# serycjon/MFT

Hardware: AMD Instinct MI355X
Metric: tracked frames/sec at 512x512, 12 RAFT iters; flow EPE vs reference (higher is better)
Workload: dtype f32 (update-block products as split fp16 x 3 on the fp16 matrix cores, fp32 accumulation; error per product <= ~2^-23, see DESIGN.md section 4 and parity below); 1 GPU; MFT.track on synthetic 512x512 video, deltas [inf,1,2,4,8,16,32], 7/7.00/7 (min/mean/max) flow pairs per timed frame, 12 RAFT iters, seeded synthetic weights (BASELINE.json configs[1]); parallelism=single GPU, frames_resident_in_hbm=True, preroll_frames=32

## Files before the change

include/mftx.h:

```cpp
#ifndef MFTX_H
#define MFTX_H

#include <stddef.h>
#include <stdint.h>

#ifdef __cplusplus
extern "C" {
#endif

#define MFTX_VERSION 400

#define MFTX_E_ARG (-1)
#define MFTX_E_ALIGN (-2)
#define MFTX_E_WORKSPACE (-3)
#define MFTX_E_STATE (-4)

#define MFTX_MAX_CANDIDATES 16

int mftx_version(void);
const char *mftx_last_error_string(void);

#define MFTX_PROFILE_CATEGORIES 14
int mftx_profile_begin(void);
int mftx_profile_end(double *ms, double *work, long long *count, int n);
// ... 31 lines not shown
    float *out; int ldo;
    int P, h, w;
    int N;
    int kh, kw;
    int act;
    float out_scale;
    const float *addend; int ld_addend;
    int stride, hin, win, pad_y, pad_x, residual_mode;
    int arith;
    int a_split, out_split;
} mftx_conv_desc;
#define MFTX_ARITH_F32 0
#define MFTX_ARITH_SPLIT 1
int mftx_conv2d(const mftx_conv_desc *d, void *stream);
int mftx_conv2d_tile(const mftx_conv_desc *d, int tile, void *stream);

int mftx_pack_tile_conv_weights(const float *wpk, int N, int taps, int cin, int cin_pad, void *wtile, void *stream);
int mftx_tile_conv2d(const mftx_conv_desc *d, const void *wtile, void *stream);
#define MFTX_OU_HEADS_WTILE_BYTES 6635520
int mftx_pack_ou_heads_weights(const float *w1pk, int cin_pad, const float *w2pk, void *wtile, void *wproj, void *stream);
int mftx_ou_heads(const float *a_split, int lda, int P, int h, int w, const void *wtile, const float *b1, const void *wproj, const float *b2,
                  float *T, float *out, int ld_out, void *stream);
int mftx_gru_half(const float *h_in, int ld_hin, const float *motion, int ld_mo, const void *wzr, const void *wq, const float *pre_zr,
                  const float *pre_q, float *z, const float *hf_in, float *hf_out, float *h_out, int ld_hout, int P, int h, int w, int pass,
                  void *stream);
int mftx_tile_conv_fills_chip(int P, int h, int w);
#define MFTX_FLOW_HEAD_WEIGHT_BYTES 32768
int mftx_pack_flow_head_weights(const float *w2pk, void *wproj, void *stream);
int mftx_flow_head(const float *hsplit, int ld_h, int P, int h, int w, const void *wtile, const float *b1, const void *wproj,
                   const float *b2, float *T, float *delta, float *coords, void *stream);
// ... 60 lines not shown
                               const float *const *fmap2, const float *const *net, const float *const *inp,
                               const float *const *ctx_parts, const void *const *fmap1_split, const void *fmap2_split,
                               const float *flow_init, int pad_left, int pad_right, int pad_top, int pad_bottom,
                               float *flow, float *occl, float *sigma, float *packed, float *flow_lr_out,
                               void *workspace, size_t workspace_bytes, void *stream);
int mftx_volume_query_split(const float *in, void *out, long long n_floats, void *stream);

typedef struct mftx_encoder mftx_encoder;
int mftx_encoder_create(const float *const *weights, int n_weights, int instance_norm, mftx_encoder **out);
int mftx_encoder_set_split_weights(mftx_encoder *e, const void *const *split, int n);
int mftx_encoder_set_graph(mftx_encoder *e, int on);
void mftx_encoder_destroy(mftx_encoder *e);
size_t mftx_encoder_workspace_bytes(int H0, int W0);
int mftx_encoder_forward(mftx_encoder *e, const uint8_t *img, int H0, int W0, float *out0, float *out1,
                         void *workspace, size_t workspace_bytes, void *stream);
int mftx_encoder_prep(const uint8_t *img, int H0, int W0, float *out, void *stream);
size_t mftx_instance_norm_workspace_bytes(int C);
int mftx_instance_norm(float *x, int rows, int C, const float *res, int mode, int split, void *workspace,
                       size_t workspace_bytes, void *stream);

int mftx_convex_upsample(const float *flow_lr, const float *ou, int ld_ou, const float *mask,
                         int P, int h, int w,
                         int pad_left, int pad_right, int pad_top, int pad_bottom,
                         float *flow, float *occl, float *sigma, float *packed, void *stream);

int mftx_chain(const float *flowL, const float *occlL, const float *sigmaL,
               const float *flowR, const float *occlR, const float *sigmaR,
               int H, int W, float *flowO, float *occlO, float *sigmaO, void *stream);

int mftx_warp_backward(const float *flow, const float *img, int C, int H, int W, float *out, void *stream);
// ... 98 lines not shown
```

mft_amd/_lib.py:

```python
from __future__ import annotations

import ctypes as C
import os
from pathlib import Path

_HERE = Path(__file__).resolve().parent
LIB_PATH = _HERE / "libmftx.so"

MAX_CANDIDATES = 16
NUM_RAFT_WEIGHTS = 34
LOOKUP_CONVC1_WEIGHT_BYTES = 393216
FLOW_BRANCH_WEIGHT_BYTES = 352256
FLOW_HEAD_WEIGHT_BYTES = 32768
OU_HEADS_WTILE_BYTES = 6635520
SPLIT_LIMIT = 65504.0


class ConvDesc(C.Structure):
    _fields_ = [("a0", C.c_void_p), ("lda0", C.c_int), ("c0", C.c_int),
                ("a1", C.c_void_p), ("lda1", C.c_int), ("c1", C.c_int),
                ("wpk", C.c_void_p), ("bias", C.c_void_p),
                ("out", C.c_void_p), ("ldo", C.c_int),
                ("P", C.c_int), ("h", C.c_int), ("w", C.c_int),
                ("N", C.c_int), ("kh", C.c_int), ("kw", C.c_int),
# ... 10 lines not shown
    "mftx_last_error_string": (C.c_char_p, []),
    "mftx_profile_begin": (C.c_int, []),
    "mftx_profile_end": (C.c_int, [C.POINTER(C.c_double), C.POINTER(C.c_double), C.POINTER(C.c_longlong), C.c_int]),
    "mftx_corr_pyramid": (C.c_int, [C.c_void_p, C.c_void_p, C.c_int, C.c_int, C.c_int, C.c_int,
                                    C.c_void_p, C.c_void_p, C.c_void_p, C.c_void_p, C.c_void_p]),
    "mftx_corr_pyramid_split": (C.c_int, [C.c_void_p, C.c_void_p, C.c_int, C.c_int, C.c_int, C.c_int,
                                          C.c_void_p, C.c_void_p, C.c_void_p, C.c_void_p, C.c_void_p, C.c_void_p]),
    "mftx_corr_pyramid_layout": (C.c_int, [C.c_int, C.c_int, C.POINTER(C.c_longlong), C.POINTER(C.c_int)]),
    "mftx_corr_lookup": (C.c_int, [C.c_void_p] * 5 + [C.c_int] * 4 + [C.c_void_p, C.c_int, C.c_void_p]),
    "mftx_fmap_pyramid": (C.c_int, [C.c_void_p] + [C.c_int] * 4 + [C.c_void_p] * 4),
    "mftx_corr_lookup_ondemand": (C.c_int, [C.c_void_p] * 6 + [C.c_int] * 5 + [C.c_void_p, C.c_int, C.c_void_p]),
    "mftx_raft_set_ondemand": (C.c_int, [C.c_void_p, C.c_int]),
    "mftx_raft_workspace_bytes_for": (C.c_size_t, [C.c_void_p, C.c_int, C.c_int, C.c_int]),
    "mftx_conv2d": (C.c_int, [C.POINTER(ConvDesc), C.c_void_p]),
    "mftx_conv2d_tile": (C.c_int, [C.POINTER(ConvDesc), C.c_int, C.c_void_p]),
    "mftx_encoder_set_split_weights": (C.c_int, [C.c_void_p, _PP, C.c_int]),
    "mftx_raft_set_split_weights": (C.c_int, [C.c_void_p, _PP, C.c_int]),
    "mftx_raft_arith": (C.c_int, [C.c_void_p]),
    "mftx_raft_set_lookup_fused": (C.c_int, [C.c_void_p, C.c_void_p]),
    "mftx_raft_set_flow_fused": (C.c_int, [C.c_void_p, C.c_void_p]),
    "mftx_raft_set_tile_weights": (C.c_int, [C.c_void_p, _PP, C.c_int]),
    "mftx_raft_set_flow_head": (C.c_int, [C.c_void_p, C.c_void_p]),
    "mftx_raft_set_ou_heads": (C.c_int, [C.c_void_p, C.c_void_p, C.c_void_p]),
    "mftx_pack_ou_heads_weights": (C.c_int, [C.c_void_p, C.c_int, C.c_void_p, C.c_void_p, C.c_void_p, C.c_void_p]),
    "mftx_ou_heads": (C.c_int, [C.c_void_p, C.c_int, C.c_int, C.c_int, C.c_int, C.c_void_p, C.c_void_p, C.c_void_p, C.c_void_p, C.c_void_p,
                                C.c_void_p, C.c_int, C.c_void_p]),
    "mftx_pack_flow_head_weights": (C.c_int, [C.c_void_p, C.c_void_p, C.c_void_p]),
    "mftx_flow_head": (C.c_int, [C.c_void_p, C.c_int, C.c_int, C.c_int, C.c_int] + [C.c_void_p] * 8),
    "mftx_pack_tile_conv_weights": (C.c_int, [C.c_void_p, C.c_int, C.c_int, C.c_int, C.c_int, C.c_void_p, C.c_void_p]),
    "mftx_tile_conv2d": (C.c_int, [C.POINTER(ConvDesc), C.c_void_p, C.c_void_p]),
# ... 31 lines not shown
                                          C.c_void_p, C.c_size_t, C.c_void_p]),
    "mftx_raft_refine_gather_ex": (C.c_int, [C.c_void_p, C.c_int, C.c_int, C.c_int, C.c_int,
                                             _PP, _PP, _PP, _PP, _PP, _PP, C.c_void_p, C.c_void_p,
                                             C.c_int, C.c_int, C.c_int, C.c_int,
                                             C.c_void_p, C.c_void_p, C.c_void_p, C.c_void_p, C.c_void_p,
                                             C.c_void_p, C.c_size_t, C.c_void_p]),
    "mftx_raft_frame_prepare_bytes": (C.c_size_t, [C.c_int, C.c_int]),
    "mftx_raft_frame_prepare": (C.c_int, [C.c_void_p, C.c_int, C.c_int] + [C.c_void_p] * 8 + [C.c_size_t, C.c_void_p]),
    "mftx_volume_query_split": (C.c_int, [C.c_void_p, C.c_void_p, C.c_longlong, C.c_void_p]),
    "mftx_encoder_create": (C.c_int, [_PP, C.c_int, C.c_int, C.POINTER(C.c_void_p)]),
    "mftx_encoder_destroy": (None, [C.c_void_p]),
    "mftx_encoder_set_graph": (C.c_int, [C.c_void_p, C.c_int]),
    "mftx_encoder_workspace_bytes": (C.c_size_t, [C.c_int, C.c_int]),
    "mftx_encoder_forward": (C.c_int, [C.c_void_p, C.c_void_p, C.c_int, C.c_int, C.c_void_p, C.c_void_p,
                                       C.c_void_p, C.c_size_t, C.c_void_p]),
    "mftx_encoder_prep": (C.c_int, [C.c_void_p, C.c_int, C.c_int, C.c_void_p, C.c_void_p]),
    "mftx_instance_norm_workspace_bytes": (C.c_size_t, [C.c_int]),
    "mftx_instance_norm": (C.c_int, [C.c_void_p, C.c_int, C.c_int, C.c_void_p, C.c_int, C.c_int, C.c_void_p, C.c_size_t, C.c_void_p]),
    "mftx_convex_upsample": (C.c_int, [C.c_void_p, C.c_void_p, C.c_int, C.c_void_p] + [C.c_int] * 7
                             + [C.c_void_p] * 5),
    "mftx_chain": (C.c_int, [C.c_void_p] * 6 + [C.c_int, C.c_int] + [C.c_void_p] * 4),
    "mftx_warp_backward": (C.c_int, [C.c_void_p, C.c_void_p, C.c_int, C.c_int, C.c_int, C.c_void_p, C.c_void_p]),
    "mftx_select": (C.c_int, [C.c_int, _PP, _PP, _PP, C.c_float, C.c_int, C.c_int] + [C.c_void_p] * 5),
    "mftx_chain_select": (C.c_int, [C.c_int] + [_PP] * 6 + [C.c_float, C.c_int, C.c_int] + [C.c_void_p] * 5),
    "mftx_chain_select_packed": (C.c_int, [C.c_int] + [_PP] * 4 + [C.c_float, C.c_int, C.c_int] + [C.c_void_p] * 5),
    "mftx_chain_select_multi": (C.c_int, [C.c_int, C.POINTER(C.c_int)] + [_PP] * 4 + [C.c_float, C.c_int, C.c_int] + [_PP] * 4
                                + [C.c_void_p]),
    "mftx_sample_points": (C.c_int, [C.c_int, _PP, _PP, _PP, C.c_int, C.c_int, C.c_int, C.c_void_p, C.c_void_p,
                                     C.c_void_p, C.c_longlong, C.c_int, C.c_void_p]),
    "mftx_splat_forward": (C.c_int, [C.c_void_p, C.c_void_p, C.c_int, C.c_void_p, C.c_int, C.c_int, C.c_int, C.c_int, C.c_int,
# ... 67 lines not shown
```

mft_amd/csrc/common.h:

```cpp
#pragma once
#include <hip/hip_runtime.h>
#include <cstdarg>
#include <cstdio>
#include <cstdint>
#include <cstdlib>
#include "../../include/mftx.h"

namespace mftx {

void set_error(const char *fmt, ...);

inline int fail(int code, const char *fmt, ...) {
    char buf[512];
    va_list ap;
    va_start(ap, fmt);
    vsnprintf(buf, sizeof buf, fmt, ap);
    va_end(ap);
    set_error("%s", buf);
    return code;
}

inline int check_launch(const char *what) {
    hipError_t e = hipGetLastError();
    if (e != hipSuccess) {
// ... 58 lines not shown
        const _Float16 b = __builtin_bit_cast(_Float16, (unsigned short)(hi ? ll >> 16 : ll));
        return (float)a + (float)b * (1.f / 2048.f);
    };
    return make_float4(dec(h.x, l.x, 0), dec(h.x, l.x, 1), dec(h.y, l.y, 0), dec(h.y, l.y, 1));
}
__device__ __forceinline__ void store_split4v(float *row, int c, float4 v) {
    const unsigned a = split_halves(v.x), b = split_halves(v.y), cc = split_halves(v.z), d = split_halves(v.w);
    char *dst = reinterpret_cast<char *>(row) + split_row_offset(c);
    *reinterpret_cast<uint2 *>(dst) = make_uint2((a & 0xffffu) | (b << 16), (cc & 0xffffu) | (d << 16));
    *reinterpret_cast<uint2 *>(dst + 16) = make_uint2((a >> 16) | (b & 0xffff0000u), (cc >> 16) | (d & 0xffff0000u));
}
#endif
__host__ __device__ inline float relu_keep_nan(float v) { return v < 0.f ? 0.f : v; }
int launch_conv(const mftx_conv_desc &d, hipStream_t s, int tile = -1);
int launch_conv_pair(const mftx_conv_desc &a, const mftx_conv_desc &b, hipStream_t s);
struct GruEpilogue {
    int mode;
    float *hx;
    int ld_hx;
    float *z;
    float *rh;
    float *hf = nullptr;
    int ld_hf = 0;
};
int launch_conv_gru(const mftx_conv_desc &d, const GruEpilogue &g, hipStream_t s);
int launch_split_weights(const float *wpk, void *out, long long n_floats, hipStream_t s);
bool conv_small_applicable(const mftx_conv_desc &d);
int launch_conv_small(const mftx_conv_desc &d, hipStream_t s, float *accum = nullptr, int ld_accum = 0);
int launch_corr_pyramid(const float *f1, const float *f2, int P, int C, int h, int w, float *const lvl[4], hipStream_t s,
                        float *f2_split = nullptr, int tile_resident = 1);
// ... 64 lines not shown
```

mft_amd/csrc/conv_gemm.hip:

```cpp
#include "common.h"
#include "profile.h"
#include "device_prims.h"
#include <cstdlib>
#include <type_traits>

namespace mftx {

enum Arith { AR_F32 = 0, AR_SPLIT = 1, AR_PRESPLIT = 2 };

#ifdef MFTX_TIMING
__device__ unsigned long long mftx_dbg[16];
#endif
#if defined(MFTX_TIMING) && MFTX_TIMING == 1
#define STAMP(i) asm volatile("s_memtime %0" : "=s"(ts[i]))
#define MFTX_TIMING_LOOP 1
#else
#define STAMP(i)
#endif

constexpr int BK = 32;
constexpr int LDK = BK;
constexpr unsigned OOB = 0x80000000u;

enum Epi { EPI_GENERIC = 0, EPI_RELU = 1, EPI_GRU_ZR = 2, EPI_GRU_Q = 3,
// ... 1291 lines not shown
        hipError_t e = hipFuncSetAttribute(reinterpret_cast<const void *>(kern),
                                           hipFuncAttributeMaxDynamicSharedMemorySize, (int)lds);
        if (e != hipSuccess) return fail((int)e, "hipFuncSetAttribute: %s", hipGetErrorString(e));
        attr_set = true;
    }
    const long long n_virtual = 8ll * cdiv(cdiv(a.M, BM), 8) * cdiv(a.N, BN) + 8ll * cdiv(cdiv(b.M, BM), 8) * cdiv(b.N, BN);
    static const bool one_tile_per_wg = tune_env("MFTX_CONV_NONPERSISTENT", 0) != 0;
    const long long slots = one_tile_per_wg ? n_virtual : (long long)num_cus() * 4;
    dim3 grid((unsigned)(n_virtual < slots ? n_virtual : slots));
    ProfScope prof(PC_CONV_GEMM, s, 2.0 * a.M * a.N * (double)(a.kh * a.kw) * (a.c0 + a.c1) +
                                        2.0 * b.M * b.N * (double)(b.kh * b.kw) * (b.c0 + b.c1));
    hipLaunchKernelGGL(kern, grid, dim3(256), lds, s, a, b);
    return check_launch("conv_gemm pair");
}

int launch_conv_gru(const mftx_conv_desc &d, const GruEpilogue &g, hipStream_t s) {
    if (int e = validate(d)) return e;
    ConvArgs a = to_args(d);
    a.hx = g.hx; a.ld_hx = g.ld_hx; a.z = g.z; a.rh = g.rh;
    a.hf = g.hf ? g.hf : g.hx; a.ld_hf = g.hf ? g.ld_hf : g.ld_hx;
    if ((g.mode == 1 && d.N != 256) || (g.mode == 2 && d.N != 128)) return fail(MFTX_E_ARG, "gru epilogue: bad N");
    return dispatch(a, g.mode == 1 ? EPI_GRU_ZR : EPI_GRU_Q, 1, s, PC_CONV_GEMM);
}

__global__ void split_weights_kernel(const float *__restrict__ in, uint4 *__restrict__ out, long long n8) {
    const long long i = (long long)blockIdx.x * blockDim.x + threadIdx.x;
    if (i >= n8) return;
    _Float16 hi[8], lo[8];
#pragma unroll
    for (int e = 0; e < 8; ++e) {
// ... 58 lines not shown
```

mft_amd/csrc/encoder.hip:

```cpp
#include "common.h"
#include "profile.h"
#include "graph_cache.h"
#include <new>

namespace mftx {


__global__ void enc_prep_kernel(const uint8_t *__restrict__ img, int H0, int W0, int pl, int pt, int Hp, int Wp,
                                float *__restrict__ out) {
    const int xo = blockIdx.x * blockDim.x + threadIdx.x;
    const int y = blockIdx.y;
    if (xo >= Wp + 6) return;
    float4 v = make_float4(0.f, 0.f, 0.f, 0.f);
    const int x = xo - 3;
    if (x >= 0 && x < Wp) {
        const int sy = min(max(y - pt, 0), H0 - 1), sx = min(max(x - pl, 0), W0 - 1);
        const uint8_t *p = img + ((long long)sy * W0 + sx) * 3;
        v.x = 2.f * ((float)p[2] / 255.0f) - 1.0f;
        v.y = 2.f * ((float)p[1] / 255.0f) - 1.0f;
        v.z = 2.f * ((float)p[0] / 255.0f) - 1.0f;
    }
    reinterpret_cast<float4 *>(out)[(long long)y * (Wp + 6) + xo] = v;
}

// ... 174 lines not shown
    return ws;
}

}

using namespace mftx;

struct mftx_encoder {
    uint32_t magic;
    int instance_norm;
    const float *w[EC_COUNT], *b[EC_COUNT];
    const float *wg[EC_COUNT];
    int arith;
    int use_graph;
    GraphCache *graphs;
};
static constexpr uint32_t ENC_MAGIC = 0x454e4358;

extern "C" int mftx_encoder_create(const float *const *weights, int n_weights, int instance_norm, mftx_encoder **out) {
    if (!weights || !out) return fail(MFTX_E_ARG, "encoder_create: null pointer");
    const int n_conv = instance_norm ? EC_COUNT - 1 : EC_COUNT;
    if (n_weights != 2 * n_conv) return fail(MFTX_E_ARG, "encoder_create: expected %d tensors, got %d", 2 * n_conv, n_weights);
    for (int i = 0; i < n_weights; ++i)
        if (!weights[i] || !aligned16(weights[i])) return fail(MFTX_E_ALIGN, "encoder_create: tensor %d null or unaligned", i);
    mftx_encoder *e = new (std::nothrow) mftx_encoder;
    if (!e) return fail(MFTX_E_ARG, "encoder_create: out of host memory");
    e->magic = ENC_MAGIC;
    e->instance_norm = instance_norm ? 1 : 0;
    for (int i = 0; i < EC_COUNT; ++i) { e->w[i] = e->wg[i] = nullptr; e->b[i] = nullptr; }
    for (int i = 0; i < n_conv; ++i) { e->w[i] = e->wg[i] = weights[2 * i]; e->b[i] = weights[2 * i + 1]; }
    e->arith = MFTX_ARITH_F32;
    e->use_graph = 1;
    e->graphs = new (std::nothrow) GraphCache;
    *out = e;
    return 0;
}

extern "C" int mftx_encoder_set_split_weights(mftx_encoder *e, const void *const *split, int n) {
    if (e && e->magic == ENC_MAGIC && e->graphs) e->graphs->clear();
    if (!e || e->magic != ENC_MAGIC) return fail(MFTX_E_STATE, "encoder_set_split_weights: bad handle");
    const int n_conv = e->instance_norm ? EC_COUNT - 1 : EC_COUNT;
    if (!split) {
        for (int i = 0; i < n_conv; ++i) e->wg[i] = e->w[i];
        e->arith = MFTX_ARITH_F32;
        return 0;
    }
    if (n != n_conv) return fail(MFTX_E_ARG, "encoder_set_split_weights: expected %d weights, got %d", n_conv, n);
    for (int i = 0; i < n_conv; ++i)
        if (!split[i] || !aligned16(split[i])) return fail(MFTX_E_ALIGN, "encoder_set_split_weights: weight %d null or unaligned", i);
    for (int i = 0; i < n_conv; ++i) e->wg[i] = static_cast<const float *>(split[i]);
    e->arith = MFTX_ARITH_SPLIT;
    return 0;
}

extern "C" void mftx_encoder_destroy(mftx_encoder *e) {
// ... 6 lines not shown
    return 0;
}

extern "C" size_t mftx_encoder_workspace_bytes(int H0, int W0) {
    if (H0 <= 0 || W0 <= 0) return 0;
    const int Hp = (H0 + 7) / 8 * 8, Wp = (W0 + 7) / 8 * 8;
    return enc_carve(nullptr, Hp, Wp).bytes;
}

namespace {
struct Enc {
    const mftx_encoder *e;
    EncWs ws;
    hipStream_t s;

    int conv(int slot, const float *in, int cin, int lda, int hin, int win, float *out, int cout, int ldo, int h,
             int w, int k, int stride, int act, const float *residual = nullptr, bool a_split = false, bool out_split = false) {
        mftx_conv_desc d{};
        d.a0 = in; d.lda0 = lda; d.c0 = cin;
        d.wpk = e->wg[slot]; d.bias = e->b[slot]; d.arith = e->arith;
        d.a_split = SP() && a_split; d.out_split = SP() && out_split;
        d.out = out; d.ldo = ldo; d.P = 1; d.h = h; d.w = w; d.N = cout; d.kh = k; d.kw = k;
        d.act = act; d.out_scale = 1.f;
        d.stride = stride; d.hin = hin; d.win = win;
        if (residual) { d.addend = residual; d.ld_addend = cout; d.residual_mode = 1; }
        ProfConvCat cat(PC_ENC_GEMM);
        return launch_conv(d, s);
    }
    bool SP() const { return e->arith == MFTX_ARITH_SPLIT; }
    int norm(float *x, int rows, int C, int mode, const float *res = nullptr) {
        return launch_instance_norm(x, rows, C, res, mode, SP() ? 1 : 0, ws.part, ws.stat, s);
    }
    int block(int c1, int c2, int ds, const float *x, int cin, int hin, int win, float *tmp, float *sc, float *out,
              int planes, int h, int w, int stride) {
        const int rows = h * w;
        if (e->instance_norm) {
            TRY(conv(c1, x, cin, cin, hin, win, tmp, planes, planes, h, w, 3, stride, 0, nullptr, true));
            TRY(norm(tmp, rows, planes, 0));
            TRY(conv(c2, tmp, planes, planes, h, w, out, planes, planes, h, w, 3, 1, 0, nullptr, true));
            const float *shortcut = x;
            if (stride != 1) {
                TRY(conv(ds, x, cin, cin, hin, win, sc, planes, planes, h, w, 1, stride, 0, nullptr, true));
// ... 23 lines not shown
    Enc E{e, enc_carve(workspace, Hp, Wp), (hipStream_t)stream};
    if (E.ws.bytes > workspace_bytes) return fail(MFTX_E_WORKSPACE, "encoder_forward: workspace %zu < %zu", workspace_bytes, E.ws.bytes);
    const bool graphs_on = e->graphs && e->use_graph && !prof_enabled();
    bool proxied = false;
    if (graphs_on && E.s == nullptr) {
        hipStream_t own = e->graphs->proxy.enter(nullptr);
        if (own) { E.s = own; proxied = true; }
    }
    struct Leave { GraphCache *g; bool on; ~Leave() { if (on) g->proxy.leave(nullptr); } } leave{e->graphs, proxied};
    hipStream_t s = E.s;
    TRY(launch_enc_prep(img, H0, W0, E.ws.img, s));
    const int h3 = Hp / 8, w3 = Wp / 8;
    auto body = [&]() -> int {
    const int h1 = Hp / 2, w1 = Wp / 2;
    {
        mftx_conv_desc d{};
        d.a0 = E.ws.img; d.lda0 = 4; d.c0 = 28;
        d.wpk = e->wg[EC_STEM]; d.bias = e->b[EC_STEM]; d.arith = e->arith;
        d.out = E.ws.a; d.ldo = 64; d.P = 1; d.h = h1; d.w = w1; d.N = 64; d.kh = 7; d.kw = 1;
        d.act = e->instance_norm ? 0 : 1; d.out_scale = 1.f;
        d.stride = 2; d.hin = Hp; d.win = Wp + 6; d.pad_y = 3; d.pad_x = -1;
        ProfConvCat cat(PC_ENC_GEMM);
        TRY(launch_conv(d, s));
    }
    if (e->instance_norm) TRY(E.norm(E.ws.a, h1 * w1, 64, 0));
    TRY(E.block(EC_L1B0C1, EC_L1B0C2, -1, E.ws.a, 64, h1, w1, E.ws.b, nullptr, E.ws.c, 64, h1, w1, 1));
    TRY(E.block(EC_L1B1C1, EC_L1B1C2, -1, E.ws.c, 64, h1, w1, E.ws.b, nullptr, E.ws.a, 64, h1, w1, 1));
    const int h2 = h1 / 2, w2 = w1 / 2;
    float *sc2 = E.ws.b + (size_t)h2 * w2 * 96;
    TRY(E.block(EC_L2B0C1, EC_L2B0C2, EC_L2B0DS, E.ws.a, 64, h1, w1, E.ws.b, sc2, E.ws.c, 96, h2, w2, 2));
    TRY(E.block(EC_L2B1C1, EC_L2B1C2, -1, E.ws.c, 96, h2, w2, E.ws.b, nullptr, E.ws.a, 96, h2, w2, 1));
    float *sc3 = E.ws.b + (size_t)h3 * w3 * 128;
    TRY(E.block(EC_L3B0C1, EC_L3B0C2, EC_L3B0DS, E.ws.a, 96, h2, w2, E.ws.b, sc3, E.ws.c, 128, h3, w3, 2));
    return E.block(EC_L3B1C1, EC_L3B1C2, -1, E.ws.c, 128, h3, w3, E.ws.b, nullptr, E.ws.a, 128, h3, w3, 1);
    };
    if (graphs_on) {
        GraphKey key{};
        key.v[0] = (uintptr_t)H0; key.v[1] = (uintptr_t)W0; key.v[2] = reinterpret_cast<uintptr_t>(workspace);
        key.v[3] = reinterpret_cast<uintptr_t>(s); key.v[4] = (uintptr_t)e->arith;
        TRY(e->graphs->run(key, s, body));
    } else {
        TRY(body());
    }
    if (e->instance_norm) return E.conv(EC_HEAD, E.ws.a, 128, 128, h3, w3, out0, 256, 256, h3, w3, 1, 1, 0, nullptr, true);
    TRY(E.conv(EC_HEAD, E.ws.a, 128, 128, h3, w3, out0, 128, 128, h3, w3, 1, 1, 3));
    return E.conv(EC_HEAD2, E.ws.a, 128, 128, h3, w3, out1, 128, 128, h3, w3, 1, 1, 1);
}

extern "C" int mftx_encoder_prep(const uint8_t *img, int H0, int W0, float *out, void *stream) {
    if (!img || !out) return fail(MFTX_E_ARG, "encoder_prep: null pointer");
    if (H0 < 1 || W0 < 1) return fail(MFTX_E_ARG, "encoder_prep: empty image");
    if (!aligned16(out)) return fail(MFTX_E_ALIGN, "encoder_prep: out must be 16-byte aligned");
    return launch_enc_prep(img, H0, W0, out, (hipStream_t)stream);
}

extern "C" size_t mftx_instance_norm_workspace_bytes(int C) {
    if (C < 8 || C > 256 || C % 8) return 0;
    return instnorm_ws_bytes(C);
}

extern "C" int mftx_instance_norm(float *x, int rows, int C, const float *res, int mode, int split, void *workspace,
                                  size_t workspace_bytes, void *stream) {
    if (!x || !workspace) return fail(MFTX_E_ARG, "instance_norm: null pointer");
// ... 15 lines not shown
```

mft_amd/csrc/raft_engine.hip:

```cpp
#include "common.h"
#include "profile.h"
#include "motion_front.h"
#include "graph_cache.h"
#include <cstdlib>
#include <new>

namespace mftx {


struct InitGather { int on; PairPtrs netp, inpp; };
struct CtxTable { const float **table; const float *own[4]; int supplied; PairPtrs parts[4]; };
__global__ void init_state_kernel(const float *__restrict__ net, const float *__restrict__ inp,
                                  const float *__restrict__ flow_init, float *hx, float *hf, float *coords1, int M, int h,
                                  int w, InitGather ga, CtxTable ct) {
    const long long i = (long long)blockIdx.x * blockDim.x + threadIdx.x;
    if (i >= (long long)M * 64) return;
    if (ct.table != nullptr && i < (long long)(M / (h * w)) * 4) {
        const int b = (int)(i >> 2), k = (int)(i & 3);
        ct.table[i] = ct.supplied ? ct.parts[k].p[b] : ct.own[k] + (long long)b * h * w * ((k & 1) ? 128 : 256);
    }
    const int m = (int)(i >> 6), q = (int)(i & 63);
    if (ga.on) {
        const int b = m / (h * w);
        net = ga.netp.p[b] - (long long)b * h * w * 128;
// ... 924 lines not shown
    if (!wpk || !out) return fail(MFTX_E_ARG, "split_weights: null pointer");
    return launch_split_weights(wpk, out, n_floats, (hipStream_t)stream);
}

extern "C" int mftx_conv2d(const mftx_conv_desc *d, void *stream) {
    if (!d) return fail(MFTX_E_ARG, "conv2d: null descriptor");
    return launch_conv(*d, (hipStream_t)stream);
}

extern "C" int mftx_conv2d_tile(const mftx_conv_desc *d, int tile, void *stream) {
    if (!d) return fail(MFTX_E_ARG, "conv2d_tile: null descriptor");
    if (tile < -1 || tile > 15) return fail(MFTX_E_ARG, "conv2d_tile: tile must be -1 (the library's choice) or 0..15");
    return launch_conv(*d, (hipStream_t)stream, tile);
}

extern "C" int mftx_convex_upsample(const float *flow_lr, const float *ou, int ld_ou, const float *mask, int P,
                                    int h, int w, int pad_left, int pad_right, int pad_top, int pad_bottom,
                                    float *flow, float *occl, float *sigma, float *packed, void *stream) {
    const bool planar = flow && occl && sigma;
    if (!flow_lr || !ou || !mask || (!planar && (flow || occl || sigma || !packed)))
        return fail(MFTX_E_ARG, "convex_upsample: null pointer (outputs: flow + occl + sigma, or packed, or both)");
    if (P <= 0 || h <= 0 || w <= 0 || ld_ou < 3) return fail(MFTX_E_ARG, "convex_upsample: bad sizes");
    return launch_convex_upsample(flow_lr, ou, ld_ou, mask, P, h, w, pad_left, pad_right, pad_top, pad_bottom, flow,
                                  occl, sigma, packed, (hipStream_t)stream);
}
```

mft_amd/ops.py:

```python
from __future__ import annotations

import ctypes as C
import math
from typing import NamedTuple

import numpy as np
import torch

from . import _lib
from ._lib import ConvDesc, MftxError, check

ACT = {None: 0, "none": 0, "relu": 1, "sigmoid": 2, "tanh": 3}


def _stream():
    return C.c_void_p(torch.cuda.current_stream().cuda_stream)


def _device_visible(t):
    return isinstance(t, torch.Tensor) and (t.is_cuda or t.is_pinned())


def copy_bytes(src: torch.Tensor, dst: torch.Tensor):
    if not (_device_visible(src) and _device_visible(dst)):
# ... 190 lines not shown
            outs = out
            want = ((h * w, 256), None) if self.instance_norm else ((h * w, 128), (h * w, 128))
            for t, shp in zip(outs, want):
                if shp is not None and (t is None or tuple(t.shape) != shp):
                    raise MftxError(f"encoder output must be {shp}")
        elif self.instance_norm:
            outs = (torch.empty(h * w, 256, dtype=torch.float32, device=self.device), None)
        else:
            outs = (torch.empty(h * w, 128, dtype=torch.float32, device=self.device),
                    torch.empty(h * w, 128, dtype=torch.float32, device=self.device))
        check(lib.mftx_encoder_forward(self._h, _chk(img_u8, "img", torch.uint8), H0, W0, _chk(outs[0], "out0"),
                                       _chk(outs[1], "out1") if outs[1] is not None else None,
                                       self._ws.data_ptr(), self._ws.numel(), _stream()), "mftx_encoder_forward")
        return outs


def encoder_prep(img_u8: torch.Tensor) -> torch.Tensor:
    lib = _lib.load()
    if img_u8.dim() != 3 or img_u8.shape[2] != 3:
        raise MftxError("encoder_prep: img must be [H0, W0, 3]")
    H0, W0 = int(img_u8.shape[0]), int(img_u8.shape[1])
    Hp, Wp = -(-H0 // 8) * 8, -(-W0 // 8) * 8
    out = torch.empty(Hp, Wp + 6, 4, dtype=torch.float32, device=img_u8.device)
    check(lib.mftx_encoder_prep(_chk(img_u8, "img", torch.uint8), H0, W0, out.data_ptr(), _stream()), "mftx_encoder_prep")
    return out


def instance_norm(x: torch.Tensor, mode: int, res: torch.Tensor = None, split: bool = False) -> torch.Tensor:
    lib = _lib.load()
    if x.dim() != 2:
# ... 230 lines not shown


def corr_lookup_ondemand(f1: torch.Tensor, f2_levels, coords: torch.Tensor, h: int, w: int, r: int = 4):
    lib = _lib.load()
    P, N, Cc = f1.shape
    out = torch.empty(P, N, 324, dtype=torch.float32, device=f1.device)
    check(lib.mftx_corr_lookup_ondemand(_chk(f1, "f1"), *[_chk(t, "f2 level") for t in f2_levels], _chk(coords, "coords"),
                                        P, Cc, h, w, r, out.data_ptr(), 324, _stream()), "mftx_corr_lookup_ondemand")
    return out


def conv2d(x: torch.Tensor, wpk: torch.Tensor, bias, P, h, w, N, kh, kw, act=None, out_scale=1.0, x2=None,
           addend=None, stride=0, hin=0, win=0, pad_y=0, pad_x=0, residual_mode=0, arith=ARITH_F32, a_split=False,
           out_split=False, out=None, tile=None, lda0=None, c0=None):
    lib = _lib.load()
    if out is None:
        out = torch.empty(P * h * w, N, dtype=torch.float32, device=x.device)
    d = ConvDesc()
    d.a0, d.lda0, d.c0 = _chk(x, "x"), x.shape[1] if lda0 is None else int(lda0), x.shape[1] if c0 is None else int(c0)
    if x2 is not None:
        d.a1, d.lda1, d.c1 = _chk(x2, "x2"), x2.shape[1], x2.shape[1]
    else:
        d.a1, d.lda1, d.c1 = None, 0, 0
    d.wpk = _chk(wpk, "wpk")
    d.bias = _chk(bias, "bias") if bias is not None else None
    d.out, d.ldo = _chk(out, "out"), out.shape[1]
    d.P, d.h, d.w, d.N, d.kh, d.kw = P, h, w, N, kh, kw
    d.act, d.out_scale = ACT[act], out_scale
    d.addend, d.ld_addend = (_chk(addend, "addend"), addend.shape[1]) if addend is not None else (None, 0)
    d.stride, d.hin, d.win, d.pad_y, d.pad_x, d.residual_mode = stride, hin, win, pad_y, pad_x, residual_mode
    d.arith = arith
    d.a_split, d.out_split = int(bool(a_split)), int(bool(out_split))
    if tile is None:
        check(lib.mftx_conv2d(C.byref(d), _stream()), "mftx_conv2d")
    else:
        check(lib.mftx_conv2d_tile(C.byref(d), int(tile), _stream()), "mftx_conv2d_tile")
    return out


def convex_upsample(flow_lr, ou, mask, P, h, w, pads=(0, 0, 0, 0), want_packed=False):
    lib = _lib.load()
    pl, pr, pt, pb = pads
    H0, W0 = 8 * h - pt - pb, 8 * w - pl - pr
    dev = flow_lr.device
    flow = torch.empty(P, 2, H0, W0, dtype=torch.float32, device=dev)
    occl = torch.empty(P, 1, H0, W0, dtype=torch.float32, device=dev)
    sigma = torch.empty(P, 1, H0, W0, dtype=torch.float32, device=dev)
    packed = torch.empty(P, H0, W0, 4, dtype=torch.float32, device=dev) if want_packed else None
    check(lib.mftx_convex_upsample(_chk(flow_lr, "flow_lr"), _chk(ou, "ou"), ou.shape[1], _chk(mask, "mask"),
                                   P, h, w, pl, pr, pt, pb, flow.data_ptr(), occl.data_ptr(), sigma.data_ptr(),
                                   packed.data_ptr() if want_packed else None, _stream()), "mftx_convex_upsample")
    return (flow, occl, sigma, packed) if want_packed else (flow, occl, sigma)
# ... 755 lines not shown
```

mft_amd/raft.py:

```python
from __future__ import annotations

import logging
import os
from pathlib import Path

import numpy as np
import torch
import torch.nn.functional as F

from . import ops
from .weights import make_weights, strip_module_prefix

logger = logging.getLogger(__name__)


def pad_amounts(H0, W0):
    ph = (((H0 // 8) + 1) * 8 - H0) % 8
    pw = (((W0 // 8) + 1) * 8 - W0) % 8
    return pw // 2, pw - pw // 2, ph // 2, ph - ph // 2


_STREAMS = {}


def _shared_stream(device, kind, index=0):
# ... 47 lines not shown
            self._build_engines()
        self._check_finite = bool(getattr(getattr(config, "raft_params", None), "check_finite", False))
        self._split_streams = int(os.environ.get("MFTX_SPLIT_STREAMS", "") or getattr(config, "split_streams", 0) or
                                  (1 if self._arith == ops.ARITH_SPLIT else 2))
        self._engines, self._side = [], []
        self._fif = self._frames_in_flight_setting(config)
        self._lanes, self._lane_next = [], 0
        self._lanes_stale = False
        self._ahead_max = max(2, int(getattr(config, "max_batches_ahead", 0) or 16))
        self._ahead = []
        self.nominal_pairs = int(getattr(config, "nominal_pairs", 0) or 7)
        self._tile_choice = {}
        fp = os.environ.get("MFTX_FRAME_PREPARE", "")
        self._frame_prepare = bool(int(fp)) if fp else bool(getattr(config, "__dict__", {}).get("frame_prepare", True))
        self._prepare_ok = {}
        self._frames = {}
        self._staging = {}
        ae = getattr(config, "__dict__", {}).get("async_encode", None)
        self._enc_waits_for_device_frames = ae is None
        if ae is None:
            ae = self._frames_in_flight_setting(config) > 1
        self._enc_stream = _shared_stream(self.device, "enc") if ae else None

    def _frames_in_flight_setting(self, config):
        return max(1, int(os.environ.get("MFTX_FRAMES_IN_FLIGHT", "") or getattr(config, "frames_in_flight", 0) or
                          (2 if self._arith == ops.ARITH_SPLIT else 1)))

    def _build_engines(self):
        graph = bool(self._engine_options.get("graph", 1))
        self.fnet_engine = ops.EncoderEngine(self.sd, "fnet", True, self.device, arith=self._arith, graph=graph)
# ... 157 lines not shown
            ring["slots"].append(slot)
        else:
            slot = ring["slots"][ring["n"] % self.STAGING_SLOTS]
        ring["n"] += 1
        if slot[1] is not None:
            slot[1].synchronize()
            slot[1] = None
        np.copyto(slot[0].numpy(), img.numpy() if img.is_contiguous() else np.ascontiguousarray(img.numpy()))
        return slot[0]

    @torch.no_grad()
    def encode(self, img_bgr, want_context=True) -> FrameFeatures:
        H0, W0 = img_bgr.shape[:2]
        img = self._device_image(img_bgr)
        h, w, pads = self._geometry(H0, W0)
        fmap, _ = self.fnet_engine.forward(img)
        net = inp = None
        if want_context:
            net, inp = self.cnet_engine.forward(img)
        return FrameFeatures(fmap, net, inp, h, w, pads, (H0, W0))

    def ensure_encode_stream(self):
        if self._enc_stream is None:
            self._enc_stream = _shared_stream(self.device, "enc")
            self._enc_stream.wait_stream(torch.cuda.current_stream(self.device))
        return self._enc_stream

    @torch.no_grad()
    def encode_packed(self, img_bgr, wait=True):
        H0, W0 = img_bgr.shape[:2]
        h, w, _ = self._geometry(H0, W0)
        N = h * w

        def run():
            img = self._device_image(img_bgr)
            buf = torch.empty(N * 512, dtype=torch.float32, device=self.device)
            self.fnet_engine.forward(img, out=(buf[: N * 256].view(N, 256), None))
            self.cnet_engine.forward(img, out=(buf[N * 256: N * 384].view(N, 128), buf[N * 384:].view(N, 128)))
            return buf

        if self._enc_stream is None or torch.cuda.current_stream(self.device) == self._enc_stream:
            cur = torch.cuda.current_stream(self.device)
            self._encode_begin(cur)
            buf = run()
            self._encode_end(cur.record_event(), cur)
            return buf, (h, w)
        main = torch.cuda.current_stream(self.device)
        self._encode_begin(self._enc_stream)
        with torch.cuda.stream(self._enc_stream):
            buf = run()
            self._encode_end(self._enc_stream.record_event(), self._enc_stream)
        if wait:
            main.wait_stream(self._enc_stream)
# ... 282 lines not shown
```

Measured before the change: 191.6 frames/s.

## Run fnet and cnet encoders together via grouped conv launches

Adds a grouped conv GEMM kernel that runs up to four independent split-arithmetic convolutions in one launch, each member taking its own virtual-tile range. A new paired encoder path interleaves the fnet and cnet layers so matching convolutions of both encoders share a launch, and the pair is captured as one graph. The aim is fewer launches and better CU fill for the small per-frame encoder convs. Members that do not fit the 64x64 tile fall back to separate launches, and the two graph caches now key on a per-encoder generation counter.

Measured after the change: 191.9 frames/s (median of 6 runs). Within noise of the previous version (+0.2%).

```diff
diff --git a/include/mftx.h b/include/mftx.h
--- a/include/mftx.h
+++ b/include/mftx.h
@@ -69,6 +69,7 @@
 #define MFTX_ARITH_SPLIT 1
 int mftx_conv2d(const mftx_conv_desc *d, void *stream);
 int mftx_conv2d_tile(const mftx_conv_desc *d, int tile, void *stream);
+int mftx_conv2d_group(const mftx_conv_desc *d, int n, void *stream);
 
 int mftx_pack_tile_conv_weights(const float *wpk, int N, int taps, int cin, int cin_pad, void *wtile, void *stream);
 int mftx_tile_conv2d(const mftx_conv_desc *d, const void *wtile, void *stream);
@@ -159,6 +160,9 @@
 size_t mftx_encoder_workspace_bytes(int H0, int W0);
 int mftx_encoder_forward(mftx_encoder *e, const uint8_t *img, int H0, int W0, float *out0, float *out1,
                          void *workspace, size_t workspace_bytes, void *stream);
+int mftx_encoder_forward_pair(mftx_encoder *fnet, mftx_encoder *cnet, const uint8_t *img, int H0, int W0, float *fmap,
+                              float *net, float *inp, void *ws_f, size_t ws_f_bytes, void *ws_c, size_t ws_c_bytes,
+                              void *stream);
 int mftx_encoder_prep(const uint8_t *img, int H0, int W0, float *out, void *stream);
 size_t mftx_instance_norm_workspace_bytes(int C);
 int mftx_instance_norm(float *x, int rows, int C, const float *res, int mode, int split, void *workspace,
diff --git a/mft_amd/_lib.py b/mft_amd/_lib.py
--- a/mft_amd/_lib.py
+++ b/mft_amd/_lib.py
@@ -48,6 +48,7 @@
     "mftx_raft_workspace_bytes_for": (C.c_size_t, [C.c_void_p, C.c_int, C.c_int, C.c_int]),
     "mftx_conv2d": (C.c_int, [C.POINTER(ConvDesc), C.c_void_p]),
     "mftx_conv2d_tile": (C.c_int, [C.POINTER(ConvDesc), C.c_int, C.c_void_p]),
+    "mftx_conv2d_group": (C.c_int, [C.POINTER(ConvDesc), C.c_int, C.c_void_p]),
     "mftx_encoder_set_split_weights": (C.c_int, [C.c_void_p, _PP, C.c_int]),
     "mftx_raft_set_split_weights": (C.c_int, [C.c_void_p, _PP, C.c_int]),
     "mftx_raft_arith": (C.c_int, [C.c_void_p]),
@@ -109,6 +110,8 @@
     "mftx_encoder_workspace_bytes": (C.c_size_t, [C.c_int, C.c_int]),
     "mftx_encoder_forward": (C.c_int, [C.c_void_p, C.c_void_p, C.c_int, C.c_int, C.c_void_p, C.c_void_p,
                                        C.c_void_p, C.c_size_t, C.c_void_p]),
+    "mftx_encoder_forward_pair": (C.c_int, [C.c_void_p, C.c_void_p, C.c_void_p, C.c_int, C.c_int, C.c_void_p, C.c_void_p,
+                                            C.c_void_p, C.c_void_p, C.c_size_t, C.c_void_p, C.c_size_t, C.c_void_p]),
     "mftx_encoder_prep": (C.c_int, [C.c_void_p, C.c_int, C.c_int, C.c_void_p, C.c_void_p]),
     "mftx_instance_norm_workspace_bytes": (C.c_size_t, [C.c_int]),
     "mftx_instance_norm": (C.c_int, [C.c_void_p, C.c_int, C.c_int, C.c_void_p, C.c_int, C.c_int, C.c_void_p, C.c_size_t, C.c_void_p]),
diff --git a/mft_amd/csrc/common.h b/mft_amd/csrc/common.h
--- a/mft_amd/csrc/common.h
+++ b/mft_amd/csrc/common.h
@@ -96,6 +96,9 @@
 __host__ __device__ inline float relu_keep_nan(float v) { return v < 0.f ? 0.f : v; }
 int launch_conv(const mftx_conv_desc &d, hipStream_t s, int tile = -1);
 int launch_conv_pair(const mftx_conv_desc &a, const mftx_conv_desc &b, hipStream_t s);
+constexpr int CONV_GROUP_MAX = 4;
+bool conv_group_member_ok(const mftx_conv_desc &d);
+int launch_conv_group(const mftx_conv_desc *d, int n, hipStream_t s);
 struct GruEpilogue {
     int mode;
     float *hx;
diff --git a/mft_amd/csrc/conv_gemm.hip b/mft_amd/csrc/conv_gemm.hip
--- a/mft_amd/csrc/conv_gemm.hip
+++ b/mft_amd/csrc/conv_gemm.hip
@@ -1329,6 +1329,60 @@
     return check_launch("conv_gemm pair");
 }
 
+struct ConvGroupArgs { ConvArgs m[CONV_GROUP_MAX]; int n; };
+
+__global__ __launch_bounds__(256, min_waves_split(1, 4))
+void conv_gemm_group_kernel(ConvGroupArgs g) {
+    int before = 0;
+#pragma unroll 1
+    for (int i = 0; i < g.n; ++i) {
+        const ConvArgs &p = g.m[i];
+        int vt = (int)blockIdx.x - before % (int)gridDim.x;
+        if (vt < 0) vt += gridDim.x;
+        if (p.a_pre) conv_gemm_body<64, 64, 2, 2, EPI_GENERIC, 32, AR_PRESPLIT, 3>(p, vt);
+        else conv_gemm_body<64, 64, 2, 2, EPI_GENERIC, 32, AR_SPLIT, 3>(p, vt);
+        before += n_virtual_tiles(p, 64, 64);
+    }
+}
+
+bool conv_group_member_ok(const mftx_conv_desc &d) {
+    if (d.arith != AR_SPLIT || d.P <= 0 || d.h <= 0 || d.w <= 0 || d.N <= 0) return false;
+    if (d.addend == nullptr && d.stride <= 1 && d.hin == 0 && conv_small_applicable(d)) return false;
+    return pick_tile(to_args(d), 1, -1) == 9;
+}
+
+int launch_conv_group(const mftx_conv_desc *d, int n, hipStream_t s) {
+    if (!d || n < 2 || n > CONV_GROUP_MAX) return fail(MFTX_E_ARG, "conv group: 2..%d members", CONV_GROUP_MAX);
+    ConvGroupArgs g{};
+    g.n = n;
+    long long n_virtual = 0;
+    double work = 0.0;
+    for (int i = 0; i < n; ++i) {
+        if (int e = validate(d[i])) return e;
+        if (!conv_group_member_ok(d[i]))
+            return fail(MFTX_E_ARG, "conv group: member %d does not run on the split arithmetic's 64 x 64 tile", i);
+        ConvArgs &a = g.m[i];
+        a = to_args(d[i]);
+        a.batch = 1;
+        n_virtual += 8ll * cdiv(cdiv(a.M, 64), 8) * cdiv(a.N, 64);
+        work += 2.0 * a.M * a.N * (double)(a.kh * a.kw) * (a.c0 + a.c1);
+    }
+    if (n_virtual > 0x7fffffffLL) return fail(MFTX_E_ARG, "conv group: too many tiles");
+    constexpr size_t lds = (size_t)3 * (64 + 64) * LDK * sizeof(float);
+    static bool attr_set = false;
+    if (!attr_set) {
+        hipError_t e = hipFuncSetAttribute(reinterpret_cast<const void *>(conv_gemm_group_kernel),
+                                           hipFuncAttributeMaxDynamicSharedMemorySize, (int)lds);
+        if (e != hipSuccess) return fail((int)e, "hipFuncSetAttribute: %s", hipGetErrorString(e));
+        attr_set = true;
+    }
+    const long long slots = (long long)num_cus() * 3;
+    dim3 grid((unsigned)(n_virtual < slots ? n_virtual : slots));
+    ProfScope prof(PC_CONV_GEMM, s, work);
+    hipLaunchKernelGGL(conv_gemm_group_kernel, grid, dim3(256), lds, s, g);
+    return check_launch("conv_gemm group");
+}
+
 int launch_conv_gru(const mftx_conv_desc &d, const GruEpilogue &g, hipStream_t s) {
     if (int e = validate(d)) return e;
     ConvArgs a = to_args(d);
diff --git a/mft_amd/csrc/encoder.hip b/mft_amd/csrc/encoder.hip
--- a/mft_amd/csrc/encoder.hip
+++ b/mft_amd/csrc/encoder.hip
@@ -1,6 +1,7 @@
 #include "common.h"
 #include "profile.h"
 #include "graph_cache.h"
+#include <atomic>
 #include <new>
 
 namespace mftx {
@@ -212,8 +213,10 @@
     int arith;
     int use_graph;
     GraphCache *graphs;
+    unsigned long long gen;
 };
 static constexpr uint32_t ENC_MAGIC = 0x454e4358;
+static unsigned long long enc_next_gen() { static std::atomic<unsigned long long> g{0}; return ++g; }
 
 extern "C" int mftx_encoder_create(const float *const *weights, int n_weights, int instance_norm, mftx_encoder **out) {
     if (!weights || !out) return fail(MFTX_E_ARG, "encoder_create: null pointer");
@@ -230,6 +233,7 @@
     e->arith = MFTX_ARITH_F32;
     e->use_graph = 1;
     e->graphs = new (std::nothrow) GraphCache;
+    e->gen = enc_next_gen();
     *out = e;
     return 0;
 }
@@ -237,6 +241,7 @@
 extern "C" int mftx_encoder_set_split_weights(mftx_encoder *e, const void *const *split, int n) {
     if (e && e->magic == ENC_MAGIC && e->graphs) e->graphs->clear();
     if (!e || e->magic != ENC_MAGIC) return fail(MFTX_E_STATE, "encoder_set_split_weights: bad handle");
+    e->gen = enc_next_gen();
     const int n_conv = e->instance_norm ? EC_COUNT - 1 : EC_COUNT;
     if (!split) {
         for (int i = 0; i < n_conv; ++i) e->wg[i] = e->w[i];
@@ -273,8 +278,9 @@
     EncWs ws;
     hipStream_t s;
 
-    int conv(int slot, const float *in, int cin, int lda, int hin, int win, float *out, int cout, int ldo, int h,
-             int w, int k, int stride, int act, const float *residual = nullptr, bool a_split = false, bool out_split = false) {
+    mftx_conv_desc desc(int slot, const float *in, int cin, int lda, int hin, int win, float *out, int cout, int ldo, int h,
+                        int w, int k, int stride, int act, const float *residual = nullptr, bool a_split = false,
+                        bool out_split = false) const {
         mftx_conv_desc d{};
         d.a0 = in; d.lda0 = lda; d.c0 = cin;
         d.wpk = e->wg[slot]; d.bias = e->b[slot]; d.arith = e->arith;
@@ -283,8 +289,22 @@
         d.act = act; d.out_scale = 1.f;
         d.stride = stride; d.hin = hin; d.win = win;
         if (residual) { d.addend = residual; d.ld_addend = cout; d.residual_mode = 1; }
+        return d;
+    }
+    int conv(int slot, const float *in, int cin, int lda, int hin, int win, float *out, int cout, int ldo, int h,
+             int w, int k, int stride, int act, const float *residual = nullptr, bool a_split = false, bool out_split = false) {
+        const mftx_conv_desc d = desc(slot, in, cin, lda, hin, win, out, cout, ldo, h, w, k, stride, act, residual, a_split, out_split);
         ProfConvCat cat(PC_ENC_GEMM);
         return launch_conv(d, s);
+    }
+    mftx_conv_desc stem_desc(const float *img, int Hp, int Wp) const {
+        mftx_conv_desc d{};
+        d.a0 = img; d.lda0 = 4; d.c0 = 28;
+        d.wpk = e->wg[EC_STEM]; d.bias = e->b[EC_STEM]; d.arith = e->arith;
+        d.out = ws.a; d.ldo = 64; d.P = 1; d.h = Hp / 2; d.w = Wp / 2; d.N = 64; d.kh = 7; d.kw = 1;
+        d.act = e->instance_norm ? 0 : 1; d.out_scale = 1.f;
+        d.stride = 2; d.hin = Hp; d.win = Wp + 6; d.pad_y = 3; d.pad_x = -1;
+        return d;
     }
     bool SP() const { return e->arith == MFTX_ARITH_SPLIT; }
     int norm(float *x, int rows, int C, int mode, const float *res = nullptr) {
@@ -338,12 +358,7 @@
     auto body = [&]() -> int {
     const int h1 = Hp / 2, w1 = Wp / 2;
     {
-        mftx_conv_desc d{};
-        d.a0 = E.ws.img; d.lda0 = 4; d.c0 = 28;
-        d.wpk = e->wg[EC_STEM]; d.bias = e->b[EC_STEM]; d.arith = e->arith;
-        d.out = E.ws.a; d.ldo = 64; d.P = 1; d.h = h1; d.w = w1; d.N = 64; d.kh = 7; d.kw = 1;
-        d.act = e->instance_norm ? 0 : 1; d.out_scale = 1.f;
-        d.stride = 2; d.hin = Hp; d.win = Wp + 6; d.pad_y = 3; d.pad_x = -1;
+        const mftx_conv_desc d = E.stem_desc(E.ws.img, Hp, Wp);
         ProfConvCat cat(PC_ENC_GEMM);
         TRY(launch_conv(d, s));
     }
@@ -371,6 +386,100 @@
     return E.conv(EC_HEAD2, E.ws.a, 128, 128, h3, w3, out1, 128, 128, h3, w3, 1, 1, 1);
 }
 
+namespace {
+struct EncPair {
+    Enc F, C;
+    hipStream_t s;
+
+    int group(const mftx_conv_desc *d, int n) {
+        ProfConvCat cat(PC_ENC_GEMM);
+        bool ok = n >= 2;
+        for (int i = 0; i < n; ++i) ok = ok && conv_group_member_ok(d[i]);
+        if (ok) return launch_conv_group(d, n, s);
+        for (int i = 0; i < n; ++i) TRY(launch_conv(d[i], s));
+        return 0;
+    }
+    int block(int c1, int c2, int ds, float *EncWs::*x, int cin, int hin, int win, size_t sc_off, float *EncWs::*out, int planes,
+              int h, int w, int stride) {
+        const int rows = h * w;
+        const float *xf = F.ws.*x, *xc = C.ws.*x;
+        float *tf = F.ws.b, *tc = C.ws.b, *sf = F.ws.b + sc_off, *sc = C.ws.b + sc_off, *of = F.ws.*out, *oc = C.ws.*out;
+        mftx_conv_desc d[4];
+        int n = 0;
+        d[n++] = F.desc(c1, xf, cin, cin, hin, win, tf, planes, planes, h, w, 3, stride, 0, nullptr, true);
+        d[n++] = C.desc(c1, xc, cin, cin, hin, win, tc, planes, planes, h, w, 3, stride, 1, nullptr, false, true);
+        if (stride != 1) {
+            d[n++] = F.desc(ds, xf, cin, cin, hin, win, sf, planes, planes, h, w, 1, stride, 0, nullptr, true);
+            d[n++] = C.desc(ds, xc, cin, cin, hin, win, sc, planes, planes, h, w, 1, stride, 0);
+        }
+        TRY(group(d, n));
+        TRY(F.norm(tf, rows, planes, 0));
+        d[0] = F.desc(c2, tf, planes, planes, h, w, of, planes, planes, h, w, 3, 1, 0, nullptr, true);
+        d[1] = C.desc(c2, tc, planes, planes, h, w, oc, planes, planes, h, w, 3, 1, 1, stride != 1 ? sc : xc, true);
+        TRY(group(d, 2));
+        if (stride != 1) TRY(F.norm(sf, rows, planes, 2));
+        return F.norm(of, rows, planes, 1, stride != 1 ? sf : xf);
+    }
+};
+}
+
+extern "C" int mftx_encoder_forward_pair(mftx_encoder *f, mftx_encoder *c, const uint8_t *img, int H0, int W0, float *fmap,
+                                         float *net, float *inp, void *ws_f, size_t ws_f_bytes, void *ws_c, size_t ws_c_bytes,
+                                         void *stream) {
+    if (!f || f->magic != ENC_MAGIC || !c || c->magic != ENC_MAGIC) return fail(MFTX_E_STATE, "encoder_forward_pair: bad handle");
+    if (!f->instance_norm || c->instance_norm) return fail(MFTX_E_ARG, "encoder_forward_pair: fnet (instance norm) first, then cnet");
+    if (f->arith != MFTX_ARITH_SPLIT || c->arith != MFTX_ARITH_SPLIT)
+        return fail(MFTX_E_ARG, "encoder_forward_pair: both encoders must run the split arithmetic");
+    if (!img || !fmap || !net || !inp || !ws_f || !ws_c) return fail(MFTX_E_ARG, "encoder_forward_pair: null pointer");
+    if (ws_f == ws_c) return fail(MFTX_E_ARG, "encoder_forward_pair: the two workspaces must differ");
+    if (H0 < 16 || W0 < 16) return fail(MFTX_E_ARG, "encoder_forward_pair: image too small");
+    if ((reinterpret_cast<uintptr_t>(ws_f) | reinterpret_cast<uintptr_t>(ws_c)) & 255)
+        return fail(MFTX_E_ALIGN, "encoder_forward_pair: workspaces must be 256-byte aligned");
+    if (prof_enabled()) {
+        TRY(mftx_encoder_forward(f, img, H0, W0, fmap, nullptr, ws_f, ws_f_bytes, stream));
+        return mftx_encoder_forward(c, img, H0, W0, net, inp, ws_c, ws_c_bytes, stream);
+    }
+    const int Hp = enc_pad(H0, W0).Hp, Wp = enc_pad(H0, W0).Wp;
+    EncPair P{Enc{f, enc_carve(ws_f, Hp, Wp), (hipStream_t)stream}, Enc{c, enc_carve(ws_c, Hp, Wp), (hipStream_t)stream}, (hipStream_t)stream};
+    if (P.F.ws.bytes > ws_f_bytes || P.C.ws.bytes > ws_c_bytes)
+        return fail(MFTX_E_WORKSPACE, "encoder_forward_pair: workspace %zu / %zu < %zu", ws_f_bytes, ws_c_bytes, P.F.ws.bytes);
+    const bool graphs_on = f->graphs && f->use_graph && c->use_graph;
+    bool proxied = false;
+    if (graphs_on && P.s == nullptr) {
+        hipStream_t own = f->graphs->proxy.enter(nullptr);
+        if (own) { P.s = P.F.s = P.C.s = own; proxied = true; }
+    }
+    struct Leave { GraphCache *g; bool on; ~Leave() { if (on) g->proxy.leave(nullptr); } } leave{f->graphs, proxied};
+    hipStream_t s = P.s;
+    TRY(launch_enc_prep(img, H0, W0, P.F.ws.img, s));
+    const int h1 = Hp / 2, w1 = Wp / 2, h2 = h1 / 2, w2 = w1 / 2, h3 = Hp / 8, w3 = Wp / 8;
+    auto body = [&]() -> int {
+        mftx_conv_desc d[2] = {P.F.stem_desc(P.F.ws.img, Hp, Wp), P.C.stem_desc(P.F.ws.img, Hp, Wp)};
+        TRY(P.group(d, 2));
+        TRY(P.F.norm(P.F.ws.a, h1 * w1, 64, 0));
+        TRY(P.block(EC_L1B0C1, EC_L1B0C2, -1, &EncWs::a, 64, h1, w1, 0, &EncWs::c, 64, h1, w1, 1));
+        TRY(P.block(EC_L1B1C1, EC_L1B1C2, -1, &EncWs::c, 64, h1, w1, 0, &EncWs::a, 64, h1, w1, 1));
+        TRY(P.block(EC_L2B0C1, EC_L2B0C2, EC_L2B0DS, &EncWs::a, 64, h1, w1, (size_t)h2 * w2 * 96, &EncWs::c, 96, h2, w2, 2));
+        TRY(P.block(EC_L2B1C1, EC_L2B1C2, -1, &EncWs::c, 96, h2, w2, 0, &EncWs::a, 96, h2, w2, 1));
+        TRY(P.block(EC_L3B0C1, EC_L3B0C2, EC_L3B0DS, &EncWs::a, 96, h2, w2, (size_t)h3 * w3 * 128, &EncWs::c, 128, h3, w3, 2));
+        return P.block(EC_L3B1C1, EC_L3B1C2, -1, &EncWs::c, 128, h3, w3, 0, &EncWs::a, 128, h3, w3, 1);
+    };
+    if (graphs_on) {
+        GraphKey key{};
+        key.v[0] = (uintptr_t)H0; key.v[1] = (uintptr_t)W0; key.v[2] = reinterpret_cast<uintptr_t>(ws_f);
+        key.v[3] = reinterpret_cast<uintptr_t>(s); key.v[4] = (uintptr_t)f->arith;
+        key.v[5] = reinterpret_cast<uintptr_t>(c); key.v[6] = (uintptr_t)c->gen; key.v[7] = reinterpret_cast<uintptr_t>(ws_c);
+        key.v[8] = 1;
+        TRY(f->graphs->run(key, s, body));
+    } else {
+        TRY(body());
+    }
+    mftx_conv_desc d[3] = {P.F.desc(EC_HEAD, P.F.ws.a, 128, 128, h3, w3, fmap, 256, 256, h3, w3, 1, 1, 0, nullptr, true),
+                           P.C.desc(EC_HEAD, P.C.ws.a, 128, 128, h3, w3, net, 128, 128, h3, w3, 1, 1, 3),
+                           P.C.desc(EC_HEAD2, P.C.ws.a, 128, 128, h3, w3, inp, 128, 128, h3, w3, 1, 1, 1)};
+    return P.group(d, 3);
+}
+
 extern "C" int mftx_encoder_prep(const uint8_t *img, int H0, int W0, float *out, void *stream) {
     if (!img || !out) return fail(MFTX_E_ARG, "encoder_prep: null pointer");
     if (H0 < 1 || W0 < 1) return fail(MFTX_E_ARG, "encoder_prep: empty image");
diff --git a/mft_amd/csrc/raft_engine.hip b/mft_amd/csrc/raft_engine.hip
--- a/mft_amd/csrc/raft_engine.hip
+++ b/mft_amd/csrc/raft_engine.hip
@@ -962,6 +962,11 @@
     return launch_conv(*d, (hipStream_t)stream, tile);
 }
 
+extern "C" int mftx_conv2d_group(const mftx_conv_desc *d, int n, void *stream) {
+    if (!d) return fail(MFTX_E_ARG, "conv2d_group: null descriptors");
+    return launch_conv_group(d, n, (hipStream_t)stream);
+}
+
 extern "C" int mftx_convex_upsample(const float *flow_lr, const float *ou, int ld_ou, const float *mask, int P,
                                     int h, int w, int pad_left, int pad_right, int pad_top, int pad_bottom,
                                     float *flow, float *occl, float *sigma, float *packed, void *stream) {
diff --git a/mft_amd/encoder_pair.py b/mft_amd/encoder_pair.py
--- /dev/null
+++ b/mft_amd/encoder_pair.py
@@ -0,0 +1,37 @@
+import torch
+
+from . import _lib
+from ._lib import ConvDesc, MftxError, check
+from .ops import ARITH_SPLIT, EncoderEngine, _chk, _conv_desc, _stream
+
+
+def encoder_pair_ok(fnet: EncoderEngine, cnet: EncoderEngine) -> bool:
+    return (fnet is not None and cnet is not None and fnet.instance_norm and not cnet.instance_norm
+            and fnet.arith == ARITH_SPLIT and cnet.arith == ARITH_SPLIT and fnet.device == cnet.device)
+
+
+def encoder_forward_pair(fnet: EncoderEngine, cnet: EncoderEngine, img_u8: torch.Tensor, out=None):
+    lib = _lib.load()
+    if not encoder_pair_ok(fnet, cnet):
+        raise MftxError("encoder_forward_pair: needs fnet (instance norm) and cnet (batch norm), both on the split arithmetic")
+    H0, W0 = img_u8.shape[:2]
+    h, w = -(-H0 // 8), -(-W0 // 8)
+    shapes = ((h * w, 256), (h * w, 128), (h * w, 128))
+    if out is None:
+        out = tuple(torch.empty(*shp, dtype=torch.float32, device=fnet.device) for shp in shapes)
+    for t, shp in zip(out, shapes):
+        if t is None or tuple(t.shape) != shp:
+            raise MftxError(f"encoder output must be {shp}")
+    ws_f, ws_c = fnet._workspace(H0, W0), cnet._workspace(H0, W0)
+    check(lib.mftx_encoder_forward_pair(fnet._h, cnet._h, _chk(img_u8, "img", torch.uint8), H0, W0, _chk(out[0], "fmap"),
+                                        _chk(out[1], "net"), _chk(out[2], "inp"), ws_f.data_ptr(), ws_f.numel(),
+                                        ws_c.data_ptr(), ws_c.numel(), _stream()), "mftx_encoder_forward_pair")
+    return tuple(out)
+
+
+def conv2d_group(members):
+    lib = _lib.load()
+    built = [_conv_desc(**m) for m in members]
+    arr = (ConvDesc * len(built))(*[d for d, _ in built])
+    check(lib.mftx_conv2d_group(arr, len(built), _stream()), "mftx_conv2d_group")
+    return [o for _, o in built]
diff --git a/mft_amd/ops.py b/mft_amd/ops.py
--- a/mft_amd/ops.py
+++ b/mft_amd/ops.py
@@ -228,6 +228,12 @@
                                        self._ws.data_ptr(), self._ws.numel(), _stream()), "mftx_encoder_forward")
         return outs
 
+    def _workspace(self, H0, W0):
+        need = _lib.load().mftx_encoder_workspace_bytes(H0, W0)
+        if self._ws is None or self._ws.numel() < need:
+            self._ws = torch.empty(need, dtype=torch.uint8, device=self.device)
+        return self._ws
+
 
 def encoder_prep(img_u8: torch.Tensor) -> torch.Tensor:
     lib = _lib.load()
@@ -488,6 +494,18 @@
            addend=None, stride=0, hin=0, win=0, pad_y=0, pad_x=0, residual_mode=0, arith=ARITH_F32, a_split=False,
            out_split=False, out=None, tile=None, lda0=None, c0=None):
     lib = _lib.load()
+    d, out = _conv_desc(x, wpk, bias, P, h, w, N, kh, kw, act, out_scale, x2, addend, stride, hin, win, pad_y, pad_x,
+                        residual_mode, arith, a_split, out_split, out, lda0, c0)
+    if tile is None:
+        check(lib.mftx_conv2d(C.byref(d), _stream()), "mftx_conv2d")
+    else:
+        check(lib.mftx_conv2d_tile(C.byref(d), int(tile), _stream()), "mftx_conv2d_tile")
+    return out
+
+
+def _conv_desc(x, wpk, bias, P, h, w, N, kh, kw, act=None, out_scale=1.0, x2=None, addend=None, stride=0, hin=0, win=0,
+               pad_y=0, pad_x=0, residual_mode=0, arith=ARITH_F32, a_split=False, out_split=False, out=None, lda0=None,
+               c0=None):
     if out is None:
         out = torch.empty(P * h * w, N, dtype=torch.float32, device=x.device)
     d = ConvDesc()
@@ -505,11 +523,7 @@
     d.stride, d.hin, d.win, d.pad_y, d.pad_x, d.residual_mode = stride, hin, win, pad_y, pad_x, residual_mode
     d.arith = arith
     d.a_split, d.out_split = int(bool(a_split)), int(bool(out_split))
-    if tile is None:
-        check(lib.mftx_conv2d(C.byref(d), _stream()), "mftx_conv2d")
-    else:
-        check(lib.mftx_conv2d_tile(C.byref(d), int(tile), _stream()), "mftx_conv2d_tile")
-    return out
+    return d, out
 
 
 def convex_upsample(flow_lr, ou, mask, P, h, w, pads=(0, 0, 0, 0), want_packed=False):
diff --git a/mft_amd/raft.py b/mft_amd/raft.py
--- a/mft_amd/raft.py
+++ b/mft_amd/raft.py
@@ -8,7 +8,7 @@
 import torch
 import torch.nn.functional as F
 
-from . import ops
+from . import encoder_pair, ops
 from .weights import make_weights, strip_module_prefix
 
 logger = logging.getLogger(__name__)
@@ -86,6 +86,7 @@
         fp = os.environ.get("MFTX_FRAME_PREPARE", "")
         self._frame_prepare = bool(int(fp)) if fp else bool(getattr(config, "__dict__", {}).get("frame_prepare", True))
         self._prepare_ok = {}
+        self._encoder_pair = bool(getattr(config, "__dict__", {}).get("encoder_pair", True))
         self._frames = {}
         self._staging = {}
         ae = getattr(config, "__dict__", {}).get("async_encode", None)
@@ -273,6 +274,9 @@
         H0, W0 = img_bgr.shape[:2]
         img = self._device_image(img_bgr)
         h, w, pads = self._geometry(H0, W0)
+        if want_context and self._encoder_pair and encoder_pair.encoder_pair_ok(self.fnet_engine, self.cnet_engine):
+            fmap, net, inp = encoder_pair.encoder_forward_pair(self.fnet_engine, self.cnet_engine, img)
+            return FrameFeatures(fmap, net, inp, h, w, pads, (H0, W0))
         fmap, _ = self.fnet_engine.forward(img)
         net = inp = None
         if want_context:
@@ -294,8 +298,12 @@
         def run():
             img = self._device_image(img_bgr)
             buf = torch.empty(N * 512, dtype=torch.float32, device=self.device)
-            self.fnet_engine.forward(img, out=(buf[: N * 256].view(N, 256), None))
-            self.cnet_engine.forward(img, out=(buf[N * 256: N * 384].view(N, 128), buf[N * 384:].view(N, 128)))
+            fmap, net, inp = buf[: N * 256].view(N, 256), buf[N * 256: N * 384].view(N, 128), buf[N * 384:].view(N, 128)
+            if self._encoder_pair and encoder_pair.encoder_pair_ok(self.fnet_engine, self.cnet_engine):
+                encoder_pair.encoder_forward_pair(self.fnet_engine, self.cnet_engine, img, out=(fmap, net, inp))
+                return buf
+            self.fnet_engine.forward(img, out=(fmap, None))
+            self.cnet_engine.forward(img, out=(net, inp))
             return buf
 
         if self._enc_stream is None or torch.cuda.current_stream(self.device) == self._enc_stream:
```
